# norabelrose/sparse-vae

Hardware: AMD Instinct MI355X
Metric: training tokens/sec + ELBO match vs CPU ref, 512-tok seq, 1/2/4/8 MI355X (higher is better)
Workload: dtype bf16; 1 GPU; c2: TransformerVAE 6L d512 heads 8 seq 512, batch 64/GPU, dense attention, dropout 0.1, fwd+bwd+allreduce+clip+RAdam; model=TransformerVAE-6L-d512, global_batch=64, seq_len=512, parallelism=dp1

## Files before the change

include/svae.h:

```cpp
#ifndef SVAE_H
#define SVAE_H
#include <stdint.h>
#ifdef __cplusplus
extern "C" {
#endif

typedef void* svae_stream_t;

enum svae_epi {
  SVAE_EPI_BF16 = 0,
  SVAE_EPI_F32 = 1,
  SVAE_EPI_F32_ACC = 2,
  SVAE_EPI_F32_ATOMIC = 3,
  SVAE_EPI_GELU = 4,
  SVAE_EPI_GELU_BWD = 5,
  SVAE_EPI_DROPOUT_RESID = 6,
  SVAE_EPI_ROTARY_BF16 = 7,
  SVAE_EPI_CE_STATS = 8,
  SVAE_EPI_CE_PROB = 9,
  SVAE_EPI_ROWSCALE_GATHER = 10
};

typedef struct svae_gemm_desc {
  const void* A;
// ... 9 lines not shown
  const float* resid;
  int64_t ldr;
  void* aux;
  int64_t ldaux;
  float alpha;
  float drop_p;
  uint64_t seed;
  const float* rot_tab;
  int32_t rot_cols, rot_d, rot_seq;
  const int32_t* labels;
  float* label_logit;
  float* a_rowsum;
  const float* k_weight;
  const float* row_a;
  const float* row_b;
  const void* gather;
  int64_t ldg;
  float* delta;
  const float* delta_o32;
  int64_t ld_o32;
  int32_t delta_hd, delta_seq;
} svae_gemm_desc;

int svae_gemm(const svae_gemm_desc* d, svae_stream_t stream);

int svae_gemm_pair(const svae_gemm_desc* d0, const svae_gemm_desc* d1, svae_stream_t stream);

#define SVAE_GROUP_MAX 256
#define SVAE_GROUP_MAX_BLOCKS 1024
int64_t svae_gemm_group_table_bytes(int32_t n);
int svae_gemm_group(const svae_gemm_desc* d, int32_t n, int32_t max_blocks, void* table, void* table_host,
                    int64_t table_bytes, svae_stream_t stream);

int svae_resid_ln_fwd(const float* x, const void* y, int32_t y_dtype, int64_t ldy, float drop_p, uint64_t seed,
                      const float* zrows, int32_t zmod, const float* w, const float* b, float* xo, void* h, float* mean,
                      float* rstd, int32_t rows, int32_t D, svae_stream_t stream);
int svae_layernorm_fwd(const void* x, int32_t x_dtype, const float* w, const float* b, void* y,
                       float* mean, float* rstd, int32_t rows, int32_t D, svae_stream_t stream);
int svae_layernorm_bwd(const void* dy, const void* x, int32_t x_dtype, const float* w, const float* mean,
                       const float* rstd, const float* dres, float* dx, void* dx_bf, float* part,
                       int32_t nblk, int32_t rows, int32_t D, int32_t zero_mod, svae_stream_t stream);
int svae_layernorm_bwd_drop(const void* dy, const void* x, int32_t x_dtype, const float* w, const float* mean,
                            const float* rstd, const float* dres, float* dx, void* dx_bf, float* part, int32_t nblk,
                            int32_t rows, int32_t D, int32_t zero_mod, float bf_drop_p, uint64_t bf_seed,
                            int32_t bf_zero_mod, float* zrow, void* zrow_bf, svae_stream_t stream);
int svae_layernorm_bwd_gelu(const void* dy, const void* x, int32_t x_dtype, const float* w, const float* mean,
                            const float* rstd, const void* gp, void* out_bf, float* part, int32_t nblk, int32_t rows,
                            int32_t D, svae_stream_t stream);
int svae_layernorm_fwd_z(float* x, const float* zrows, int32_t zmod, const float* w, const float* b, void* y,
                         float* mean, float* rstd, int32_t rows, int32_t D, svae_stream_t stream);
int svae_layernorm_nblk(int32_t rows);
#define SVAE_LN_MULTI_MAX 4
int svae_layernorm_fwd_multi(const float* x, const float* const* w, const float* const* b, void* const* y, int32_t n,
                             float* mean, float* rstd, int32_t rows, int32_t D, svae_stream_t stream);
int svae_layernorm_bwd_multi(const void* const* dy, const float* x, const float* const* w, const float* mean,
                             const float* rstd, const float* dres, float* dx, float* const* part, int32_t nblk,
                             int32_t n, int32_t rows, int32_t D, svae_stream_t stream);

int svae_colsum(const void* in, int32_t in_dtype, int32_t rows, int32_t cols, int64_t ld, float* out,
                int32_t accumulate, svae_stream_t stream);

#define SVAE_COLSUM_MAX 8
typedef struct svae_colsum_seg {
  const float* in;
  float* out;
  int64_t ld;
// ... 238 lines not shown
```

sparse-vae_amd/csrc/gemm.hip:

```cpp
#include "common.h"
#include "../../include/svae.h"
#include <string.h>
#include <algorithm>
#include <vector>

using namespace svae;

namespace {

constexpr int BM = 128, BN = 128, BK = 64;
constexpr int TILE_BYTES = BM * BK * 2;

struct GP {
  const bf16* A; const bf16* B;
  long long lda, ldb, sA, sB;
  int M, N, K, splits, kchunk, tiles_n, tiles_m;
  void* C; long long ldc, sC;
  const float* bias;
  const float* resid; long long ldr;
  void* aux; long long ldaux;
  float alpha, drop_p;
  unsigned long long seed;
  const float* rot_tab; int rot_cols, rot_d, rot_seq;
  const int* labels; float* label_logit;
// ... 1406 lines not shown

struct SlabRed {
  const float* slab;
  float* C;
  int M, N;
  long long ldc;
  int splits;
};
__device__ __forceinline__ void slab_reduce_range(const SlabRed& r, int blk, int nblk) {
  const int N4 = r.N / 4;
  const long long total = (long long)r.M * N4, plane = (long long)r.M * r.N;
  for (long long i = (long long)blk * 256 + threadIdx.x; i < total; i += (long long)nblk * 256) {
    const long long m = i / N4;
    const int n = (int)(i - m * N4) * 4;
    const float* src = r.slab + m * r.N + n;
    f32x4 acc = *(const f32x4*)src;
    for (int s = 1; s < r.splits; ++s) acc += *(const f32x4*)(src + s * plane);
    f32x4* dst = (f32x4*)(r.C + m * r.ldc + n);
    *dst = *dst + acc;
  }
}
__global__ __launch_bounds__(256) void slab_reduce_kernel(SlabRed r) { slab_reduce_range(r, blockIdx.x, gridDim.x); }
__global__ __launch_bounds__(256) void slab_reduce2_kernel(SlabRed r0, SlabRed r1, int nb0) {
  if ((int)blockIdx.x < nb0) slab_reduce_range(r0, blockIdx.x, nb0);
  else slab_reduce_range(r1, blockIdx.x - nb0, (int)gridDim.x - nb0);
}
struct alignas(16) SlabRedSlot {
  SlabRed r;
};
__global__ __launch_bounds__(256) void slab_reduce_list_kernel(const SlabRedSlot* __restrict__ list, int n) {
  for (int e = 0; e < n; ++e) {
    const SlabRed r = load_uniform(&list[e].r);
    slab_reduce_range(r, blockIdx.x, gridDim.x);
  }
}

}

static SlabRed slab_red(const svae_gemm_desc* d) {
  return SlabRed{(const float*)d->aux, (float*)d->C, d->M, d->N, (long long)d->ldc, d->splits};
}
static long long slab_blocks(const svae_gemm_desc* d) {
  return std::min(4096LL, ((long long)d->M * (d->N / 4) + 255) / 256);
}
static int launch_slab_reduce(const svae_gemm_desc* d, hipStream_t s) {
  hipLaunchKernelGGL(slab_reduce_kernel, dim3((unsigned)slab_blocks(d)), dim3(256), 0, s, slab_red(d));
  SVAE_LAUNCH_CHECK();
  return SVAE_OK;
}

static int validate_desc(const svae_gemm_desc* d) {
  if (!d || !d->A || !d->B || (!d->C && d->epi != SVAE_EPI_CE_STATS)) return SVAE_EINVAL;
  const bool epi_new = d->epi == SVAE_EPI_CE_PROB || d->epi == SVAE_EPI_ROWSCALE_GATHER;
  if (d->M <= 0 || d->N <= 0 || d->K <= 0 || d->batch <= 0 || d->splits <= 0) return SVAE_EINVAL;
  if ((d->K % 8 && !(d->a_t && d->b_t)) || d->lda % 8 || d->ldb % 8) return SVAE_EINVAL;
  if (d->a_t && d->M % 8) return SVAE_EINVAL;
  if (d->b_t && d->N % 8) return SVAE_EINVAL;
  if (((uintptr_t)d->A | (uintptr_t)d->B) & 15) return SVAE_EINVAL;
  if (d->batch_stride_a % 8 || d->batch_stride_b % 8) return SVAE_EINVAL;
  if (d->epi < 0 || d->epi > SVAE_EPI_ROWSCALE_GATHER) return SVAE_EINVAL;
  if (epi_new && (d->a_t || d->splits != 1 || d->batch != 1 || !d->labels || !d->row_a)) return SVAE_EINVAL;
  if (d->epi == SVAE_EPI_CE_PROB && !d->aux) return SVAE_EINVAL;
  if (d->epi == SVAE_EPI_ROWSCALE_GATHER &&
      (!d->row_b || !d->gather || d->ldg % 8 || ((uintptr_t)d->gather & 15) || d->N % 8))
    return SVAE_EINVAL;
  if (d->k_weight && (!d->a_rowsum || !d->a_t || (d->splits != 1 && !(d->epi == SVAE_EPI_F32_ATOMIC && d->aux))))
// ... 404 lines not shown
  memcpy(img.data(), &h, sizeof(h));
  memcpy(img.data() + o_gp, gp.data(), (size_t)n * sizeof(GPSlot));
  if (!map[0].empty()) memcpy(img.data() + o_ma, map[0].data(), map[0].size() * sizeof(GMap));
  if (!map[1].empty()) memcpy(img.data() + o_mb, map[1].data(), map[1].size() * sizeof(GMap));
  if (!red.empty()) memcpy(img.data() + o_red, red.data(), red.size() * sizeof(SlabRedSlot));
  hipStream_t s = (hipStream_t)stream;
  if (memcmp(table_host, img.data(), (size_t)bytes) != 0) {
    memcpy(table_host, img.data(), (size_t)bytes);
    if (hipMemcpyAsync(table, table_host, (size_t)bytes, hipMemcpyHostToDevice, s) != hipSuccess ||
        hipStreamSynchronize(s) != hipSuccess) {
      memset(table_host, 0, sizeof(GroupHeader));
      return SVAE_ELAUNCH;
    }
  }
  const char* t = (const char*)table;
  const GPSlot* tab = (const GPSlot*)(t + o_gp);
  if (!map[0].empty()) {
    hipLaunchKernelGGL((gemm256_group_kernel<SVAE_EPI_F32_ACC>), dim3((unsigned)map[0].size()), dim3(512), 0, s, tab,
                       (const GMap*)(t + o_ma));
    SVAE_LAUNCH_CHECK();
  }
  if (!map[1].empty()) {
    hipLaunchKernelGGL((gemm256_group_kernel<G3_EPI_SLAB>), dim3((unsigned)map[1].size()), dim3(512), 0, s, tab,
                       (const GMap*)(t + o_mb));
    SVAE_LAUNCH_CHECK();
    const long long rb = std::max(1LL, std::min(2048LL, (red_elems + 255) / 256));
    hipLaunchKernelGGL(slab_reduce_list_kernel, dim3((unsigned)rb), dim3(256), 0, s, (const SlabRedSlot*)(t + o_red),
                       (int)red.size());
    SVAE_LAUNCH_CHECK();
  }
  return SVAE_OK;
}

#ifdef SVAE_STAMPS
extern "C" __attribute__((visibility("default"))) int svae_debug_stamps(unsigned long long* host) {
  return hipMemcpyFromSymbol(host, HIP_SYMBOL(svae_stamps), sizeof(svae_stamps)) == hipSuccess ? 0 : -1;
}
extern "C" __attribute__((visibility("default"))) int svae_debug_rt(unsigned long long* host) {
  return hipMemcpyFromSymbol(host, HIP_SYMBOL(svae_rt), sizeof(svae_rt)) == hipSuccess ? 0 : -1;
}
extern "C" __attribute__((visibility("default"))) int svae_debug_stamps_clear() {
  static unsigned long long zeros[8 * 96 * 3];
  return hipMemcpyToSymbol(HIP_SYMBOL(svae_stamps), zeros, sizeof(zeros)) == hipSuccess ? 0 : -1;
}
#endif
```

sparse-vae_amd/sparse_vae/_native.py:

```python
import ctypes
import os

import torch

_HERE = os.path.dirname(os.path.abspath(__file__))
LIB_PATH = os.environ.get('SVAE_LIB') or os.path.join(_HERE, 'libsvae.so')

c_void_p, c_int32, c_int64, c_float, c_uint64 = (ctypes.c_void_p, ctypes.c_int32, ctypes.c_int64,
                                                  ctypes.c_float, ctypes.c_uint64)
c_fptr = ctypes.c_void_p

EPI_BF16, EPI_F32, EPI_F32_ACC, EPI_F32_ATOMIC, EPI_GELU, EPI_GELU_BWD, EPI_DROPOUT_RESID, \
    EPI_ROTARY_BF16, EPI_CE_STATS, EPI_CE_PROB, EPI_ROWSCALE_GATHER = range(11)

LATENT_L2, LATENT_COSINE, LATENT_KL = range(3)
LATENT_METRICS = {'l2': LATENT_L2, 'cosine': LATENT_COSINE, 'kl': LATENT_KL}
LATENT_MAX_BLOCKS = 1024
TSNE_ROWS_PER_BLOCK, TSNE_TILE_COLS = 512, 256
PAIR_RBF, PAIR_IMQ = range(2)
PAIR_KINDS = {'rbf': PAIR_RBF, 'imq': PAIR_IMQ}
PAIRSUM_TILE_COLS, PAIRSUM_MAX_P, MMD_REDUCE_BLOCKS = 32, 8, 256
KMEANS_MAX_K, KMEANS_TILE_CENTROIDS, KMEANS_SORT_BLOCKS, KMEANS_SEED_BLOCK_ROWS = 1024, 32, 256, 256


# ... 10 lines not shown
        ('bias', c_void_p), ('resid', c_void_p), ('ldr', c_int64),
        ('aux', c_void_p), ('ldaux', c_int64),
        ('alpha', c_float), ('drop_p', c_float), ('seed', c_uint64),
        ('rot_tab', c_void_p), ('rot_cols', c_int32), ('rot_d', c_int32), ('rot_seq', c_int32),
        ('labels', c_void_p), ('label_logit', c_void_p),
        ('a_rowsum', c_void_p),
        ('k_weight', c_void_p), ('row_a', c_void_p), ('row_b', c_void_p), ('gather', c_void_p), ('ldg', c_int64),
        ('delta', c_void_p), ('delta_o32', c_void_p), ('ld_o32', c_int64), ('delta_hd', c_int32), ('delta_seq', c_int32),
    ]


class AttnDesc(ctypes.Structure):
    _fields_ = [
        ('q', c_void_p), ('k', c_void_p), ('v', c_void_p), ('o', c_void_p),
        ('sq', c_int64), ('sk', c_int64), ('sv', c_int64), ('so', c_int64),
        ('bq', c_int64), ('bk', c_int64), ('bv', c_int64), ('bo', c_int64),
        ('key_pad', c_void_p), ('lse', c_void_p),
        ('B', c_int32), ('H', c_int32), ('Lq', c_int32), ('Lk', c_int32), ('hd', c_int32), ('causal', c_int32),
        ('scale', c_float),
        ('dout', c_void_p), ('sdo', c_int64), ('bdo', c_int64),
        ('delta', c_void_p), ('dq', c_void_p), ('bdq', c_int64),
        ('dk', c_void_p), ('dv', c_void_p),
        ('sdk', c_int64), ('sdv', c_int64), ('bdk', c_int64), ('bdv', c_int64),
        ('rot_tab', c_void_p), ('rot_d', c_int32),
        ('o32', c_void_p), ('so32', c_int64), ('bo32', c_int64),
        ('dq_part', c_void_p), ('dq_bf', c_void_p), ('ldq_bf', c_int64),
        ('window', c_int32),
        ('delta_ready', c_int32),
        ('o_lo', c_void_p), ('so_lo', c_int64), ('bo_lo', c_int64),
        ('fwd_ws', c_void_p), ('fwd_ws_elems', c_int64),
    ]


GROUP_MAX = 256
COLSUM_MAX = 8
LN_MULTI_MAX = 4


ZPROJ_MAX = 32


class ZprojSeg(ctypes.Structure):
    _fields_ = [('g', c_void_p), ('W', c_void_p), ('dW', c_void_p), ('db', c_void_p)]


class ZprojFwdSeg(ctypes.Structure):
    _fields_ = [('W', c_void_p), ('bias', c_void_p), ('out', c_void_p)]


class ColsumSeg(ctypes.Structure):
    _fields_ = [('inp', c_void_p), ('out', c_void_p), ('ld', c_int64), ('rows', c_int32), ('cols', c_int32)]


_SIGS = {
    'svae_gemm': [ctypes.POINTER(GemmDesc), c_void_p],
    'svae_gemm_pair': [ctypes.POINTER(GemmDesc), ctypes.POINTER(GemmDesc), c_void_p],
    'svae_gemm_group_table_bytes': [c_int32],
    'svae_gemm_group': [ctypes.POINTER(GemmDesc), c_int32, c_int32, c_void_p, c_void_p, c_int64, c_void_p],
    'svae_resid_ln_fwd': [c_void_p, c_void_p, c_int32, c_int64, c_float, c_uint64, c_void_p, c_int32, c_void_p,
                          c_void_p, c_void_p, c_void_p, c_void_p, c_void_p, c_int32, c_int32, c_void_p],
    'svae_layernorm_fwd': [c_void_p, c_int32, c_void_p, c_void_p, c_void_p, c_void_p, c_void_p, c_int32, c_int32,
                           c_void_p],
    'svae_layernorm_bwd': [c_void_p, c_void_p, c_int32, c_void_p, c_void_p, c_void_p, c_void_p, c_void_p, c_void_p,
                           c_void_p, c_int32, c_int32, c_int32, c_int32, c_void_p],
    'svae_layernorm_bwd_drop': [c_void_p, c_void_p, c_int32, c_void_p, c_void_p, c_void_p, c_void_p, c_void_p,
                                c_void_p, c_void_p, c_int32, c_int32, c_int32, c_int32, c_float, c_uint64, c_int32,
                                c_void_p, c_void_p, c_void_p],
    'svae_layernorm_bwd_gelu': [c_void_p, c_void_p, c_int32, c_void_p, c_void_p, c_void_p, c_void_p, c_void_p,
                                c_void_p, c_int32, c_int32, c_int32, c_void_p],
    'svae_layernorm_nblk': [c_int32],
    'svae_colsum': [c_void_p, c_int32, c_int32, c_int32, c_int64, c_void_p, c_int32, c_void_p],
    'svae_colsum_multi': [c_void_p, c_int32, c_void_p],
    'svae_attn_fwd': [ctypes.POINTER(AttnDesc), c_void_p],
    'svae_attn_bwd': [ctypes.POINTER(AttnDesc), c_void_p],
    'svae_attn_dq_part_elems': [c_int32, c_int32, c_int32, c_int32, c_int32],
    'svae_attn_dq_part_elems_w': [c_int32, c_int32, c_int32, c_int32, c_int32, c_int32],
    'svae_attn_fwd_ws_elems': [c_int32, c_int32, c_int32, c_int32, c_int32, c_int32, c_int32],
    'svae_transpose_blocks': [c_void_p, c_void_p, c_void_p, c_int32, c_int32, c_void_p],
    'svae_dq_finalize': [c_void_p, c_void_p, c_int64, c_int32, c_int32, c_void_p, c_int32, c_void_p],
    'svae_embedding_fwd': [c_void_p, c_void_p, c_void_p, c_void_p, c_int32, c_int32, c_void_p],
    'svae_embedding_fwd_dual': [c_void_p, c_void_p, c_void_p, c_void_p, c_int32, c_int32, c_void_p],
    'svae_embedding_bwd': [c_void_p, c_void_p, c_void_p, c_int32, c_int32, c_void_p],
    'svae_reparam_kl_fwd': [c_void_p, c_void_p, c_uint64, c_void_p, c_void_p, c_void_p, c_void_p, c_void_p,
                            c_void_p, c_int32, c_int32, c_void_p],
    'svae_reparam_kl_bwd': [c_void_p, c_void_p, c_void_p, c_void_p, c_void_p, c_void_p, c_int32, c_int32, c_void_p],
    'svae_ce_finalize': [c_void_p, c_int32, c_void_p, c_void_p, c_int32, c_int32, c_int32, c_int32, c_void_p,
                         c_void_p, c_void_p, c_void_p, c_void_p, c_void_p],
    'svae_ce_weighted_nll': [c_void_p, c_void_p, c_void_p, c_int32, c_int32, c_int32, c_int32, c_void_p, c_void_p,
                             c_void_p],
    'svae_ce_red_ws_elems': [c_int32],
# ... 135 lines not shown
```

sparse-vae_amd/sparse_vae/engine.py:

```python
import math
import os
from collections import OrderedDict

import torch

from . import kernels as K
from ._native import COLSUM_MAX, GROUP_MAX, LN_MULTI_MAX, ZPROJ_MAX
from ._native import EPI_BF16, EPI_F32, EPI_F32_ACC, EPI_GELU, EPI_GELU_BWD, EPI_DROPOUT_RESID, \
    EPI_ROTARY_BF16, EPI_CE_STATS, EPI_F32_ATOMIC, EPI_CE_PROB, EPI_ROWSCALE_GATHER

bf16, f32 = torch.bfloat16, torch.float32
ALIGN = 64
CE_CHUNK_NUMEL = 2 ** 30


def _attn_entries(pre, d, learned):
    out = []
    if learned:
        out.append((pre + 'learned_queries', (1, learned, d)))
        names = ['k_linear', 'v_linear']
    else:
        names = ['q_linear', 'k_linear', 'v_linear']
    out += [(pre + n + '.weight', (d, d)) for n in names]
    out += [(pre + n + '.bias', (d,)) for n in names]
# ... 179 lines not shown
        self.head_mode = os.environ.get('SVAE_HEAD', 'prob')
        assert self.head_mode in ('prob', 'logits'), self.head_mode
        self.dw_group = os.environ.get('SVAE_DW_GROUP', '1') != '0'
        self._dw_jobs = []
        self._dwq = None
        self._dw_names = False
        self._dwg_states, self._dwg_sched = [], {}
        self._zp_pending, self._zp_ctx = [], None
        self._cs_pending = []
        self.ncu = (torch.cuda.get_device_properties(flat.device).multi_processor_count
                    if flat.device.type == 'cuda' else 256)

    def rot(self, L, window=0):
        need = max(L, self.hp.num_latents)
        base = 2 * window * 32 if window else 10000
        t = self._rot.get(base)
        if t is None or t.shape[0] < need:
            t = rotary_table(max(need, 512), self.d, base).to(self.P.device)
            self._rot[base] = t
        return t

    def _ln_fwd(self, name, x, rows, tag, zsplice=None):
        D = self.d
        y = self.ws.get(tag + '.y', (rows, D))
        mean = self.ws.get(tag + '.mean', (rows,), f32)
        rstd = self.ws.get(tag + '.rstd', (rows,), f32)
        if zsplice is not None:
            K.layernorm_fwd_z(x, zsplice[0], zsplice[1], self.P.f(name + '.weight'), self.P.f(name + '.bias'), y, mean,
                              rstd, rows, D)
        else:
            K.layernorm_fwd(x, self.P.f(name + '.weight'), self.P.f(name + '.bias'), y, mean, rstd, rows, D)
        return y, (x, mean, rstd)

    def _ln_bwd(self, name, dy, st, rows, dres, dx, dx_bf=None, bf_drop=None, zsplice=None, gelu=None):
        x, mean, rstd = st
        D = self.d
        wg = self.P.grad[self.P.offsets[name + '.weight'][0]:][:2 * D]
        if len(self._cs_pending) == COLSUM_MAX:
            self.flush_colsum()
        k, n1 = len(self._cs_pending), 1024 * 2 * D
        part = self.ws.get('ln.parts', (COLSUM_MAX * n1,), f32)[k * n1:(k + 1) * n1]
        if gelu is not None:
            K.layernorm_bwd_gelu(dy, x, self.P.f(name + '.weight'), mean, rstd, gelu, dx_bf, wg, rows, D, part,
                                 defer=self._cs_pending)
            return
        K.layernorm_bwd(dy, x, self.P.f(name + '.weight'), mean, rstd, dres, dx, dx_bf, wg, rows, D, part,
                        bf_drop=bf_drop, zsplice=zsplice, defer=self._cs_pending)

    def flush_zproj(self):
        if self._zp_pending:
            z_bf, dz, B, d, Z = self._zp_ctx
            K.zproj_bwd_multi(self._zp_pending, z_bf, dz, B, d, Z)
            self._zp_pending = []

    def flush_colsum(self):
        if self._cs_pending:
            K.colsum_multi(self._cs_pending)
            self._cs_pending = []

    def _job(self, dY, X, wname, rows, n_out, n_in, ldy=None, ldx=None, bias=None):
        bg = None
        if bias is not None:
            off = self.P.offsets[bias][0]
            bg = self.P.grad[off:off + n_out]
        return K.DwJob(dY, X, self.P.g(wname), rows, n_out, n_in, ldy, ldx, bg)

# ... 11 lines not shown
        ncu = self.ncu
        eff = lambda s: tiles * s / (ncu * -(-(tiles * s) // ncu))
        return 2 if tiles >= ncu and eff(2) > eff(1) + 0.1 else 1

    def _dw_pair(self, j0, j1):
        if self._dwq is not None:
            self._dw(j0)
            self._dw(j1)
        else:
            K.linear_dw_pair(j0, j1)

    def _bname(self, name, st):
        return f'{name}.{st["tag"]}' if self._dw_names else name

    def flush_dw(self):
        q, self._dw_jobs = self._dw_jobs, []
        k = 0
        for c in range(0, len(q), GROUP_MAX):
            jobs = q[c:c + GROUP_MAX]
            key = tuple((j.n_out, j.n_in, j.rows) for j in jobs)
            if key not in self._dwg_sched:
                self._dwg_sched[key] = K.group_schedule(key, self.ncu)
            for idx, splits, slab in self._dwg_sched[key]:
                if len(self._dwg_states) <= k:
                    self._dwg_states.append(K.DwGroupState(self.P.device))
                K.linear_dw_group([jobs[i] for i in idx], splits, self._dwg_states[k], slab=slab)
                k += 1

    def _db(self, dY, bname, rows, cols, ld=None):
        off = self.P.offsets[bname][0]
        K.colsum(dY, rows, cols, ld or cols, self.P.grad[off:off + cols])

    def layer_fwd(self, pre, x, B, Sx, L, pad, *, learned=0, cross=False, causal=False, ctx=None, heads, hd,
                  drop_p=0.0, seed=0, tag, out=None, window=0, out_bf=None, zsplice=None, ctx_ln=None):
        d, ws, P = self.d, self.ws, self.P
        rows_x = B * Sx
        rot = self.rot(max(Sx, L), window)
        st = {'pre': pre, 'B': B, 'Sx': Sx, 'L': L, 'learned': learned, 'cross': cross, 'causal': causal,
              'heads': heads, 'hd': hd, 'drop_p': drop_p, 'seed': seed, 'x': x, 'tag': tag, 'window': window}
        a = pre + 'attention.'
        h, st['ln_a'] = self._ln_fwd(pre + 'attn_layer_norm', x, rows_x, tag + '.ln_a', zsplice=zsplice)
        st['h'] = h
        pad_k = pad if Sx == L else None
        if learned:
            Lq = learned
            kv = ws.get(tag + '.kv', (rows_x, 2 * d))
            K.gemm(h, P.w(a + 'k_linear.weight'), kv, rows_x, 2 * d, d, epi=EPI_ROTARY_BF16,
                   bias=P.f(a + 'k_linear.bias'), rot=rot, rot_cols=d, rot_d=d, rot_seq=Sx)
            q = P.w(a + 'learned_queries').view(Lq, d)
            qargs = dict(sq=d, bq=0)
            kt, vt, sk = kv, kv[:, d:], 2 * d
            st['kv'] = kv
        else:
            Lq = Sx
            qkv = ws.get(tag + '.qkv', (rows_x, 3 * d))
            K.gemm(h, P.w(a + 'q_linear.weight'), qkv, rows_x, 3 * d, d, epi=EPI_ROTARY_BF16,
                   bias=P.f(a + 'q_linear.bias'), rot=rot, rot_cols=2 * d, rot_d=d, rot_seq=Sx)
            q = qkv
            qargs = dict(sq=3 * d, bq=Sx * 3 * d)
            kt, vt, sk = qkv[:, d:], qkv[:, 2 * d:], 3 * d
            st['qkv'] = qkv
        rows_q = B * Lq
        O = ws.get(tag + '.O', (rows_q, d))
        Ox = self._o_extra(tag + '.O', rows_q, d, Lq)
        lse = ws.get(tag + '.lse', (B, heads, Lq), f32)
        K.attention(q, kt, vt, O, lse, B=B, H=heads, Lq=Lq, Lk=Sx, hd=hd, so=d, bo=Lq * d, sk=sk, sv=sk,
                    bk=Sx * sk, bv=Sx * sk, key_pad=pad_k, causal=causal, window=window, **Ox, **qargs)
        st.update(O=O, Ox=Ox, lse=lse, Lq=Lq, pad_k=pad_k)
        resid = Lq == Sx
        x1 = ws.get(tag + '.x1', (rows_q, d), f32)
        K.gemm(O, P.w(a + 'output_linear.weight'), x1, rows_q, d, d, epi=EPI_F32,
               bias=P.f(a + 'output_linear.bias'), resid=x if resid else None, ldr=d)
        st['resid'] = resid
        st['x1'] = x1
        xc = x1
        if cross:
            c = pre + 'cross_attention.'
            rows_c = B * L
            if ctx_ln is not None:
                cx, st['ln_ctx'] = ctx_ln
                st['ctx_deferred'] = True
            else:
                cx, st['ln_ctx'] = self._ln_fwd(pre + 'context_layer_norm', ctx, rows_c, tag + '.ln_ctx')
            hq, st['ln_cross'] = self._ln_fwd(pre + 'cross_attn_layer_norm', x1, rows_q, tag + '.ln_cross')
            qc = ws.get(tag + '.qc', (rows_q, d))
            K.gemm(hq, P.w(c + 'q_linear.weight'), qc, rows_q, d, d, epi=EPI_ROTARY_BF16, bias=P.f(c + 'q_linear.bias'),
                   rot=rot, rot_cols=d, rot_d=d, rot_seq=Lq)
            kvc = ws.get(tag + '.kvc', (rows_c, 2 * d))
            K.gemm(cx, P.w(c + 'k_linear.weight'), kvc, rows_c, 2 * d, d, epi=EPI_ROTARY_BF16,
                   bias=P.f(c + 'k_linear.bias'), rot=rot, rot_cols=d, rot_d=d, rot_seq=L)
            Oc = ws.get(tag + '.Oc', (rows_q, d))
            Ocx = self._o_extra(tag + '.Oc', rows_q, d, Lq)
            lsec = ws.get(tag + '.lsec', (B, heads, Lq), f32)
            K.attention(qc, kvc, kvc[:, d:], Oc, lsec, B=B, H=heads, Lq=Lq, Lk=L, hd=hd, sq=d, bq=Lq * d, sk=2 * d,
                        sv=2 * d, bk=L * 2 * d, bv=L * 2 * d, so=d, bo=Lq * d, key_pad=pad, causal=False, **Ocx)
            st['Ocx'] = Ocx
            x2 = ws.get(tag + '.x2', (rows_q, d), f32)
            K.gemm(Oc, P.w(c + 'output_linear.weight'), x2, rows_q, d, d, epi=EPI_F32,
                   bias=P.f(c + 'output_linear.bias'), resid=x1, ldr=d)
            st.update(cx=cx, hq=hq, qc=qc, kvc=kvc, Oc=Oc, lsec=lsec, x2=x2, pad_ctx=pad)
            xc = x2
        h2, st['ln_f'] = self._ln_fwd(pre + 'ffn_layer_norm', xc, rows_q, tag + '.ln_f')
        gprime = ws.get(tag + '.gprime', (rows_q, 4 * d))
        f = ws.get(tag + '.f', (rows_q, 4 * d))
        K.gemm(h2, P.w(pre + 'ffn.0.weight'), f, rows_q, 4 * d, d, epi=EPI_GELU, bias=P.f(pre + 'ffn.0.bias'),
               aux=gprime, ldaux=4 * d)
        out = ws.get(tag + '.out', (rows_q, d), f32) if out is None else out
        K.gemm(f, P.w(pre + 'ffn.2.weight'), out, rows_q, d, 4 * d, epi=EPI_DROPOUT_RESID, resid=xc, ldr=d,
               drop_p=drop_p, seed=seed, aux=out_bf, ldaux=d if out_bf is not None else 0)
        st.update(h2=h2, gprime=gprime, f=f, xc=xc, rows_q=rows_q)
        return out, st

    def _o_extra(self, tag, rows_q, d, Lq):
        return dict(o_lo=self.ws.get(tag + 'lo', (rows_q, d)), so_lo=d, bo_lo=Lq * d)

    def _dq_part(self, B, H, Lq, Lk, hd, window=0):
        n = K.attn_dq_part_elems(B, H, Lq, Lk, hd, window)
        t = self.ws.bufs.get('b.dqpart')
        return t if t is not None and t.numel() >= n else self.ws.get('b.dqpart', (n,), f32)

    def layer_bwd(self, st, dout, dx_out, *, dx_accumulate=False, dctx=None, g2_ready=False, next_drop=None,
                  zsplice=None, next_st=None):
        d, ws, P = self.d, self.ws, self.P
        pre, B, Sx, L, Lq = st['pre'], st['B'], st['Sx'], st['L'], st['Lq']
        heads, hd = st['heads'], st['hd']
        rows_x, rows_q = B * Sx, st['rows_q']
        rot = self.rot(max(Sx, L), st['window'])
        a = pre + 'attention.'
        bn = lambda name: self._bname(name, st)
        self._dwq = self._dw_jobs if self._dw_names else None
        g2 = ws.get(bn('b.g2'), (rows_q, d))
        if not g2_ready:
            K.dropout_bwd_cast(dout, g2, st['drop_p'], st['seed'], rows_q, d)
        dpre = ws.get(bn('b.dpre'), (rows_q, 4 * d))
        K.gemm(g2, P.wT(pre + 'ffn.2.weight', d, 4 * d), dpre, rows_q, 4 * d, d, epi=EPI_GELU_BWD, aux=st['gprime'],
# ... 306 lines not shown
        gp0 = ws.get('h0_gprime', (T, d))
        h0 = ws.get('h0', (T, d))
        K.gemm(xf, P.w('output_layer.0.weight'), h0, T, d, d, epi=EPI_GELU, bias=P.f('output_layer.0.bias'),
               aux=gp0, ldaux=d)
        hh, ln_h = self._ln_fwd('output_layer.2', h0, T, 'head.ln')
        return hh, gp0, h0, ln_h

    def _decode(self, x_emb, zb, padm, B, L, dropout, seed, x_ready=False):
        hp, d, ws, P = self.hp, self.d, self.ws, self.P
        T, Z = B * L, hp.latent_depth
        if self.window and L % 32:
            raise ValueError(f'sparse decoder attention needs seq_len % 32 == 0 (SparseAttention block_size 32, '
                             f'sparse_attention.py:81), got {L}')
        xs = ws.get('x_dec0', (T, d), f32)
        if not x_ready:
            xs.copy_(x_emb)
        xf = ws.get('xf_bf', (T, d))
        dec = []
        zf_batch = d % 8 == 0 and Z <= 1024
        if zf_batch:
            zall = ws.get('zproj_all', (hp.num_layers, B, d), f32)
            segs = [(P.w(f'z_projections.{i}.weight'), P.f(f'z_projections.{i}.bias'), zall[i])
                    for i in range(hp.num_layers)]
            for c0 in range(0, len(segs), ZPROJ_MAX):
                K.zproj_fwd_multi(segs[c0:c0 + ZPROJ_MAX], zb, B, d, Z)
        for i in range(hp.num_layers):
            last = i + 1 == hp.num_layers
            if not zf_batch:
                K.gemm(zb, P.w(f'z_projections.{i}.weight'), xs, B, d, Z, ldc=L * d, epi=EPI_F32,
                       bias=P.f(f'z_projections.{i}.bias'))
            xs, st = self.layer_fwd(f'decoder_layers.{i}.', xs, B, L, L, padm, causal=True, heads=self.H,
                                    hd=self.hd, drop_p=dropout, seed=_mix_seed(seed, i), tag=f'd{i}',
                                    out=ws.get(f'x_dec{i + 1}', (T, d), f32), window=self.window,
                                    out_bf=xf if last else None, zsplice=(zall[i], L) if zf_batch else None)
            dec.append(st)
        return xf, dec

    def reconstruct_f32(self, x_emb, z, pad=None):
        hp, d, P = self.hp, self.d, self.P
        dev = P.device
        B, L = x_emb.shape[0], x_emb.shape[1]
        T, V, Z, H, hd = B * L, hp.vocab_size, hp.latent_depth, self.H, self.hd
        rot = self.rot(L, self.window)
        padm = None
        if pad is not None:
            padm = torch.empty(B, L, dtype=torch.uint8, device=dev)
            padm.copy_(pad)
        x = x_emb.reshape(T, d).clone()
        h = torch.empty(T, d, device=dev)
        qkv = torch.empty(T, 3 * d, device=dev)
        o = torch.empty(T, d, device=dev)
        x1 = torch.empty(T, d, device=dev)
        f = torch.empty(T, 4 * d, device=dev)
        for i in range(hp.num_layers):
            pre = f'decoder_layers.{i}.'
            a = pre + 'attention.'
            K.gemm_f32(z, P.f(f'z_projections.{i}.weight'), x, B, d, Z, ldc=L * d, bias=P.f(f'z_projections.{i}.bias'))
            K.layernorm_fwd_f32(x, P.f(pre + 'attn_layer_norm.weight'), P.f(pre + 'attn_layer_norm.bias'), h, T, d)
            K.gemm_f32(h, P.f(a + 'q_linear.weight'), qkv, T, 3 * d, d, epi=EPI_ROTARY_BF16, bias=P.f(a + 'q_linear.bias'),
                       rot=rot, rot_cols=2 * d, rot_d=d, rot_seq=L)
            K.attention_f32(qkv, qkv[:, d:], qkv[:, 2 * d:], o, B=B, H=H, Lq=L, Lk=L, hd=hd, sq=3 * d, sk=3 * d,
                            sv=3 * d, so=d, bq=L * 3 * d, bk=L * 3 * d, bv=L * 3 * d, bo=L * d, key_pad=padm, causal=True,
                            window=self.window)
            K.gemm_f32(o, P.f(a + 'output_linear.weight'), x1, T, d, d, bias=P.f(a + 'output_linear.bias'), resid=x, ldr=d)
            K.layernorm_fwd_f32(x1, P.f(pre + 'ffn_layer_norm.weight'), P.f(pre + 'ffn_layer_norm.bias'), h, T, d)
            K.gemm_f32(h, P.f(pre + 'ffn.0.weight'), f, T, 4 * d, d, epi=EPI_GELU, bias=P.f(pre + 'ffn.0.bias'))
            K.gemm_f32(f, P.f(pre + 'ffn.2.weight'), x, T, d, 4 * d, resid=x1, ldr=d)
# ... 161 lines not shown
```

sparse-vae_amd/sparse_vae/kernels.py:

```python
import ctypes
import os
from typing import NamedTuple

import torch

from . import _native as N
from ._native import lib, check, ptr, stream

bf16, f32 = torch.bfloat16, torch.float32

_gemm_desc = N.GemmDesc()


def _dev(*ts):
    for t in ts:
        if t is not None and not t.is_cuda:
            raise RuntimeError('libsvae kernels need device tensors (no CPU fallback)')


def gemm(A, B, C, M, N_, K, *, a_t=False, b_t=False, lda=None, ldb=None, ldc=None, epi=N.EPI_BF16, bias=None,
         resid=None, ldr=0, aux=None, ldaux=0, alpha=1.0, splits=1, drop_p=0.0, seed=0, rot=None, rot_cols=0,
         rot_d=0, rot_seq=0, labels=None, label_logit=None, batch=1, sA=0, sB=0, sC=0, a_rowsum=None, k_weight=None,
         row_a=None, row_b=None, gather=None, ldg=0, delta=None, delta_o32=None, ld_o32=0, delta_hd=0, delta_seq=0):
    d = _fill_desc(_gemm_desc, A, B, C, M, N_, K, a_t=a_t, b_t=b_t, lda=lda, ldb=ldb, ldc=ldc, epi=epi, bias=bias,
                   resid=resid, ldr=ldr, aux=aux, ldaux=ldaux, alpha=alpha, splits=splits, drop_p=drop_p, seed=seed,
                   rot=rot, rot_cols=rot_cols, rot_d=rot_d, rot_seq=rot_seq, labels=labels, label_logit=label_logit,
                   batch=batch, sA=sA, sB=sB, sC=sC, a_rowsum=a_rowsum, k_weight=k_weight, row_a=row_a, row_b=row_b,
                   gather=gather, ldg=ldg)
    if delta is not None:
        _dev(delta, delta_o32)
        assert delta.dtype == f32 and delta_o32.dtype == f32 and delta.numel() >= M * (N_ // delta_hd)
    d.delta, d.delta_o32, d.ld_o32 = ptr(delta), ptr(delta_o32), ld_o32
    d.delta_hd, d.delta_seq = delta_hd, delta_seq
    check(lib.svae_gemm(ctypes.byref(d), stream()), 'svae_gemm')


def _fill_desc(d, A, B, C, M, N_, K, *, a_t=False, b_t=False, lda=None, ldb=None, ldc=None, epi=N.EPI_BF16,
               bias=None, resid=None, ldr=0, aux=None, ldaux=0, alpha=1.0, splits=1, drop_p=0.0, seed=0, rot=None,
               rot_cols=0, rot_d=0, rot_seq=0, labels=None, label_logit=None, batch=1, sA=0, sB=0, sC=0,
               a_rowsum=None, k_weight=None, row_a=None, row_b=None, gather=None, ldg=0):
    _dev(A, B, C)
    assert A.dtype == bf16 and B.dtype == bf16
    d.A, d.B = A.data_ptr(), B.data_ptr()
    d.lda = lda if lda is not None else (M if a_t else K)
    d.ldb = ldb if ldb is not None else (N_ if b_t else K)
    d.batch_stride_a, d.batch_stride_b = sA, sB
    d.M, d.N, d.K = M, N_, K
    d.batch, d.splits = batch, splits
    d.a_t, d.b_t = int(a_t), int(b_t)
    d.epi = epi
    d.C = ptr(C)
    d.ldc = ldc if ldc is not None else N_
    d.batch_stride_c = sC
    d.bias = ptr(bias)
    d.resid = ptr(resid)
    d.ldr = ldr
    d.aux = ptr(aux)
    d.ldaux = ldaux
    d.alpha = alpha
    d.drop_p = drop_p
    d.seed = seed & 0xFFFFFFFFFFFFFFFF
    d.rot_tab = ptr(rot)
    d.rot_cols, d.rot_d, d.rot_seq = rot_cols, rot_d, rot_seq
    d.labels = ptr(labels)
    d.label_logit = ptr(label_logit)
    d.a_rowsum = ptr(a_rowsum)
    d.k_weight = ptr(k_weight)
# ... 1002 lines not shown
```

Before: 2.830 million tokens/s.

## Fuse decoder attention output projection with residual add and FFN LayerNorm

Adds a persistent GEMM kernel for N=512 where each block owns full 128x512 output rows. It adds bias and residual, then computes LayerNorm mean and rstd through cross-wave LDS reductions and writes the normalized bf16 activations in the epilogue. In the decoder layers this replaces the separate output-linear GEMM plus LayerNorm launch, saving one pass over the f32 activations and a kernel launch. The cost is a new hand-written GEMM with BK=32 and one block per CU, which may run the matmul itself less efficiently than the existing tuned GEMM.

```diff
diff --git a/include/svae.h b/include/svae.h
--- a/include/svae.h
+++ b/include/svae.h
@@ -65,6 +65,18 @@
 int svae_gemm_group(const svae_gemm_desc* d, int32_t n, int32_t max_blocks, void* table, void* table_host,
                     int64_t table_bytes, svae_stream_t stream);
 
+typedef struct svae_ln_tail {
+  const float* ln_w;
+  const float* ln_b;
+  void* h;
+  float* mean;
+  float* rstd;
+  const float* zrows;
+  int32_t zmod;
+  int32_t max_blocks;
+} svae_ln_tail;
+int svae_gemm_ln(const svae_gemm_desc* d, const svae_ln_tail* t, svae_stream_t stream);
+
 int svae_resid_ln_fwd(const float* x, const void* y, int32_t y_dtype, int64_t ldy, float drop_p, uint64_t seed,
                       const float* zrows, int32_t zmod, const float* w, const float* b, float* xo, void* h, float* mean,
                       float* rstd, int32_t rows, int32_t D, svae_stream_t stream);
diff --git a/sparse-vae_amd/csrc/gemm.hip b/sparse-vae_amd/csrc/gemm.hip
--- a/sparse-vae_amd/csrc/gemm.hip
+++ b/sparse-vae_amd/csrc/gemm.hip
@@ -1462,6 +1462,234 @@
   for (int e = 0; e < n; ++e) {
     const SlabRed r = load_uniform(&list[e].r);
     slab_reduce_range(r, blockIdx.x, gridDim.x);
+  }
+}
+
+constexpr int GL_BK = 32;
+constexpr int GL_TA = 128 * GL_BK * 2;
+constexpr int GL_TB = 512 * GL_BK * 2;
+constexpr int GL_STAGE = GL_TA + GL_TB;
+constexpr int GL_NSTAGE = 3;
+constexpr int GL_SIDE = 3 * 512 * 4 + 128 * 2 * 8 * 4;
+constexpr int GL_PIECES = 5;
+static_assert(8 * 1024 == GL_TA && 8 * 4 * 1024 == GL_TB, "8 waves x (1 + 4) pieces cover a stage exactly");
+static_assert(GL_NSTAGE * GL_STAGE + GL_SIDE <= 160 * 1024, "LDS");
+
+struct LNTail {
+  const float* w; const float* b;
+  bf16* h; float* mean; float* rstd;
+  const float* zrows; int zmod;
+};
+
+__device__ __forceinline__ void gl_piece(int piece, int lane, int& row, int& c) {
+  const int slot = piece * 64 + lane;
+  row = slot >> 2;
+  c = (slot & 3) ^ ((row >> 1) & 3);
+}
+
+__device__ __forceinline__ void gl_issue(const GP& p, int m0, int k0, char* stage, int wave, int offa,
+                                         const int (&offb)[4]) {
+  const int krem = p.K - k0;
+  const u32x4 ra = buffer_rsrc(p.A + (long long)m0 * p.lda + k0, 0x7FFFFFF0u);
+  const u32x4 rb = buffer_rsrc(p.B + k0, 0x7FFFFFF0u);
+  if (krem >= GL_BK && m0 + 128 <= p.M) {
+    dma16_lds(ra, stage + wave * 1024, offa);
+  } else {
+    int row, c;
+    gl_piece(wave, lane_id_fresh(), row, c);
+    const bool ok = row < p.M - m0 && c * 8 < krem;
+    dma16_lds(ra, stage + wave * 1024, ok ? (row * (int)p.lda + c * 8) * 2 : 0x7FFFFFF0);
+  }
+  if (krem >= GL_BK) {
+    dma16x4_lds(rb, stage + GL_TA + wave * 4096, offb[0], offb[1], offb[2], offb[3]);
+  } else {
+    const int lane = lane_id_fresh();
+    int o[4];
+#pragma unroll
+    for (int i = 0; i < 4; ++i) {
+      int row, c;
+      gl_piece(wave * 4 + i, lane, row, c);
+      o[i] = c * 8 < krem ? (row * (int)p.ldb + c * 8) * 2 : 0x7FFFFFF0;
+    }
+    dma16x4_lds(rb, stage + GL_TA + wave * 4096, o[0], o[1], o[2], o[3]);
+  }
+}
+
+template <int EPI, bool LN>
+__global__ __launch_bounds__(512, 1) void gemm_ln_kernel(GP p, LNTail t) {
+  __shared__ __attribute__((aligned(16))) char ring[GL_NSTAGE * GL_STAGE + GL_SIDE];
+  float* sbias = (float*)(ring + GL_NSTAGE * GL_STAGE);
+  float* slw = sbias + 512;
+  float* slb = sbias + 1024;
+  float* sstat = sbias + 1536;
+  const int tid = threadIdx.x, lane = tid & 63;
+  const int wave = __builtin_amdgcn_readfirstlane(tid >> 6);
+  const int g = lane >> 4, li = lane & 15;
+  const int step_m = (int)gridDim.x * 128;
+  int m0 = (int)blockIdx.x * 128;
+  if (m0 >= p.M) return;
+  sbias[tid] = p.bias ? p.bias[tid] : 0.f;
+  if constexpr (LN) {
+    slw[tid] = t.w[tid];
+    slb[tid] = t.b[tid];
+  }
+  const int nk = (p.K + GL_BK - 1) / GL_BK;
+  int offa, offb[4];
+  {
+    int row, c;
+    gl_piece(wave, lane, row, c);
+    offa = (row * (int)p.lda + c * 8) * 2;
+#pragma unroll
+    for (int i = 0; i < 4; ++i) {
+      gl_piece(wave * 4 + i, lane, row, c);
+      offb[i] = (row * (int)p.ldb + c * 8) * 2;
+    }
+  }
+  int pm0 = m0, pkt = 0, is = 0, ahead = 0;
+  auto issue = [&]() {
+    if (pm0 >= p.M) return;
+    gl_issue(p, pm0, pkt * GL_BK, ring + is * GL_STAGE, wave, offa, offb);
+    is = is + 1 == GL_NSTAGE ? 0 : is + 1;
+    ++ahead;
+    if (++pkt == nk) {
+      pkt = 0;
+      pm0 += step_m;
+    }
+  };
+  issue();
+  issue();
+  int cs = 0;
+  bool drained = false;
+  const int aoff = li * 64 + ((g ^ ((li >> 1) & 3)) << 4);
+  for (; m0 < p.M; m0 += step_m) {
+    f32x4 acc[8][4];
+#pragma unroll
+    for (int i = 0; i < 8; ++i)
+#pragma unroll
+      for (int j = 0; j < 4; ++j) acc[i][j] = (f32x4){0.f, 0.f, 0.f, 0.f};
+    for (int kt = 0; kt < nk; ++kt) {
+      if (ahead >= 2 && !drained) asm volatile("s_waitcnt vmcnt(%0)" ::"n"(GL_PIECES) : "memory");
+      else asm volatile("s_waitcnt vmcnt(0)" ::: "memory");
+      drained = false;
+      __builtin_amdgcn_s_barrier();
+      issue();
+      const char* la = ring + cs * GL_STAGE + aoff;
+      const char* lb = la + GL_TA + wave * 64 * 64;
+      bf16x8 af[8], bfr[4];
+#pragma unroll
+      for (int i = 0; i < 8; ++i) af[i] = *(const bf16x8*)(la + i * 1024);
+#pragma unroll
+      for (int j = 0; j < 4; ++j) bfr[j] = *(const bf16x8*)(lb + j * 1024);
+#pragma unroll
+      for (int i = 0; i < 8; ++i)
+#pragma unroll
+        for (int j = 0; j < 4; ++j) acc[i][j] = mfma16(bfr[j], af[i], acc[i][j]);
+      cs = cs + 1 == GL_NSTAGE ? 0 : cs + 1;
+      --ahead;
+    }
+    drained = true;
+    const int nb = wave * 64;
+    f32x4 b4[4];
+    if constexpr (EPI != SVAE_EPI_DROPOUT_RESID) {
+#pragma unroll
+      for (int j = 0; j < 4; ++j) b4[j] = *(const f32x4*)(sbias + nb + j * 16 + 4 * g);
+    }
+    const bool ld = p.resid != nullptr;
+    auto ld_row = [&](int i, f32x4 (&r)[4]) {
+      const int m = m0 + i * 16 + li;
+#pragma unroll
+      for (int j = 0; j < 4; ++j)
+        r[j] = (ld && m < p.M) ? *(const f32x4*)(p.resid + (long long)m * p.ldr + nb + j * 16 + 4 * g)
+                               : (f32x4){0.f, 0.f, 0.f, 0.f};
+    };
+    f32x4 cur[4], nxt[4];
+    ld_row(0, cur);
+#pragma unroll
+    for (int i = 0; i < 8; ++i) {
+      if (i + 1 < 8) ld_row(i + 1, nxt);
+      const int rl = i * 16 + li, m = m0 + rl;
+      f32x4 x[4];
+#pragma unroll
+      for (int j = 0; j < 4; ++j) {
+        if constexpr (EPI == SVAE_EPI_DROPOUT_RESID) {
+          x[j] = acc[i][j];
+          if (p.drop_p > 0.f) dropout4(p, x[j], m, nb + j * 16 + 4 * g);
+        } else {
+          x[j] = acc[i][j] + b4[j];
+        }
+        x[j] += cur[j];
+      }
+      if (t.zrows && m < p.M && m % t.zmod == 0) {
+        const float* z = t.zrows + (long long)(m / t.zmod) * 512 + nb + 4 * g;
+#pragma unroll
+        for (int j = 0; j < 4; ++j) x[j] = *(const f32x4*)(z + j * 16);
+      }
+      store_rows_f32((float*)p.C, p.ldc, m0 + i * 16, p.M, nb, 512, x, g, li);
+      if constexpr (EPI == SVAE_EPI_DROPOUT_RESID) {
+        if (p.aux) store_rows_bf16<false>((bf16*)p.aux, p.ldaux, m0 + i * 16, p.M, nb, 512, x, g, li);
+      }
+      if constexpr (LN) {
+        float s = 0.f;
+#pragma unroll
+        for (int j = 0; j < 4; ++j) {
+          acc[i][j] = x[j];
+          s += (x[j][0] + x[j][1]) + (x[j][2] + x[j][3]);
+        }
+        s = sum_x16_x32(s);
+        if (g == 0) sstat[rl * 16 + wave] = s;
+      }
+      if (i + 1 < 8) {
+#pragma unroll
+        for (int j = 0; j < 4; ++j) cur[j] = nxt[j];
+      }
+    }
+    if constexpr (LN) {
+      auto row_total = [&](int i, int which) {
+        const float* s = sstat + (i * 16 + li) * 16 + which * 8;
+        const f32x4 a = *(const f32x4*)s, b = *(const f32x4*)(s + 4);
+        return ((a[0] + a[1]) + (a[2] + a[3])) + ((b[0] + b[1]) + (b[2] + b[3]));
+      };
+      asm volatile("s_waitcnt lgkmcnt(0)" ::: "memory");
+      __builtin_amdgcn_s_barrier();
+      float mean[8], rstd[8];
+#pragma unroll
+      for (int i = 0; i < 8; ++i) {
+        mean[i] = row_total(i, 0) * (1.0f / 512.0f);
+        float sq = 0.f;
+#pragma unroll
+        for (int j = 0; j < 4; ++j)
+#pragma unroll
+          for (int e = 0; e < 4; ++e) {
+            const float d = acc[i][j][e] - mean[i];
+            sq += d * d;
+          }
+        sq = sum_x16_x32(sq);
+        if (g == 0) sstat[(i * 16 + li) * 16 + 8 + wave] = sq;
+      }
+      asm volatile("s_waitcnt lgkmcnt(0)" ::: "memory");
+      __builtin_amdgcn_s_barrier();
+      f32x4 w4[4], l4[4];
+#pragma unroll
+      for (int j = 0; j < 4; ++j) {
+        w4[j] = *(const f32x4*)(slw + nb + j * 16 + 4 * g);
+        l4[j] = *(const f32x4*)(slb + nb + j * 16 + 4 * g);
+      }
+#pragma unroll
+      for (int i = 0; i < 8; ++i) {
+        rstd[i] = rsqrtf(row_total(i, 1) * (1.0f / 512.0f) + 1e-5f);
+        f32x4 y[4];
+#pragma unroll
+        for (int j = 0; j < 4; ++j)
+#pragma unroll
+          for (int e = 0; e < 4; ++e) y[j][e] = (acc[i][j][e] - mean[i]) * rstd[i] * w4[j][e] + l4[j][e];
+        store_rows_bf16<false>(t.h, 512, m0 + i * 16, p.M, nb, 512, y, g, li);
+        const int m = m0 + i * 16 + li;
+        if (wave == 0 && g == 0 && m < p.M) {
+          t.mean[m] = mean[i];
+          t.rstd[m] = rstd[i];
+        }
+      }
+    }
   }
 }
 
@@ -1932,6 +2160,37 @@
   return SVAE_OK;
 }
 
+SVAE_EXPORT int svae_gemm_ln(const svae_gemm_desc* d, const svae_ln_tail* t, svae_stream_t stream) {
+  if (!d || !t) return SVAE_EINVAL;
+  if (const int rc = validate_desc(d)) return rc;
+  if (d->N != 512 || d->a_t || d->b_t || d->batch != 1 || d->splits != 1 || d->alpha != 1.0f) return SVAE_EINVAL;
+  if (d->epi != SVAE_EPI_F32 && d->epi != SVAE_EPI_DROPOUT_RESID) return SVAE_EINVAL;
+  if (d->a_rowsum || d->k_weight || d->delta) return SVAE_EINVAL;
+  if ((d->epi == SVAE_EPI_F32 && d->aux) || (d->epi == SVAE_EPI_DROPOUT_RESID && d->bias)) return SVAE_EINVAL;
+  if (!(d->drop_p >= 0.f && d->drop_p < 1.f)) return SVAE_EINVAL;
+  if (d->ldc % 4 || d->ldc < 512 || ((uintptr_t)d->C & 15) || d->lda < d->K || d->ldb < d->K || d->lda > (1 << 22) ||
+      d->ldb > (1 << 20) || d->M > (1 << 30) || (d->resid && d->ldr < 512) || (d->aux && d->ldaux < 512))
+    return SVAE_EINVAL;
+  const bool ln = t->ln_w != nullptr;
+  if (ln && (!t->ln_b || !t->h || !t->mean || !t->rstd || ((uintptr_t)t->h & 15) || ((uintptr_t)t->ln_w & 3) ||
+             ((uintptr_t)t->ln_b & 3) || ((uintptr_t)t->mean & 3) || ((uintptr_t)t->rstd & 3)))
+    return SVAE_EINVAL;
+  if (!ln && (d->epi != SVAE_EPI_F32 || t->ln_b || t->h || t->mean || t->rstd)) return SVAE_EINVAL;
+  if (t->zrows && (t->zmod <= 0 || ((uintptr_t)t->zrows & 15))) return SVAE_EINVAL;
+  if (t->max_blocks < 0) return SVAE_EINVAL;
+  GP p;
+  fill_gp(d, p);
+  const LNTail lt{t->ln_w, t->ln_b, (bf16*)t->h, t->mean, t->rstd, t->zrows, t->zmod};
+  const int tiles = (d->M + 127) / 128;
+  const dim3 grid((unsigned)std::min(tiles, t->max_blocks ? t->max_blocks : device_cus()));
+  hipStream_t s = (hipStream_t)stream;
+  if (!ln) hipLaunchKernelGGL((gemm_ln_kernel<SVAE_EPI_F32, false>), grid, dim3(512), 0, s, p, lt);
+  else if (d->epi == SVAE_EPI_F32) hipLaunchKernelGGL((gemm_ln_kernel<SVAE_EPI_F32, true>), grid, dim3(512), 0, s, p, lt);
+  else hipLaunchKernelGGL((gemm_ln_kernel<SVAE_EPI_DROPOUT_RESID, true>), grid, dim3(512), 0, s, p, lt);
+  SVAE_LAUNCH_CHECK();
+  return SVAE_OK;
+}
+
 #ifdef SVAE_STAMPS
 extern "C" __attribute__((visibility("default"))) int svae_debug_stamps(unsigned long long* host) {
   return hipMemcpyFromSymbol(host, HIP_SYMBOL(svae_stamps), sizeof(svae_stamps)) == hipSuccess ? 0 : -1;
diff --git a/sparse-vae_amd/sparse_vae/_native.py b/sparse-vae_amd/sparse_vae/_native.py
--- a/sparse-vae_amd/sparse_vae/_native.py
+++ b/sparse-vae_amd/sparse_vae/_native.py
@@ -66,6 +66,11 @@
     ]
 
 
+class LnTail(ctypes.Structure):
+    _fields_ = [('ln_w', c_void_p), ('ln_b', c_void_p), ('h', c_void_p), ('mean', c_void_p), ('rstd', c_void_p),
+                ('zrows', c_void_p), ('zmod', c_int32), ('max_blocks', c_int32)]
+
+
 GROUP_MAX = 256
 COLSUM_MAX = 8
 LN_MULTI_MAX = 4
@@ -90,6 +95,7 @@
     'svae_gemm': [ctypes.POINTER(GemmDesc), c_void_p],
     'svae_gemm_pair': [ctypes.POINTER(GemmDesc), ctypes.POINTER(GemmDesc), c_void_p],
     'svae_gemm_group_table_bytes': [c_int32],
+    'svae_gemm_ln': [ctypes.POINTER(GemmDesc), c_void_p, c_void_p],
     'svae_gemm_group': [ctypes.POINTER(GemmDesc), c_int32, c_int32, c_void_p, c_void_p, c_int64, c_void_p],
     'svae_resid_ln_fwd': [c_void_p, c_void_p, c_int32, c_int64, c_float, c_uint64, c_void_p, c_int32, c_void_p,
                           c_void_p, c_void_p, c_void_p, c_void_p, c_void_p, c_int32, c_int32, c_void_p],
diff --git a/sparse-vae_amd/sparse_vae/engine.py b/sparse-vae_amd/sparse_vae/engine.py
--- a/sparse-vae_amd/sparse_vae/engine.py
+++ b/sparse-vae_amd/sparse_vae/engine.py
@@ -235,6 +235,14 @@
             K.layernorm_fwd(x, self.P.f(name + '.weight'), self.P.f(name + '.bias'), y, mean, rstd, rows, D)
         return y, (x, mean, rstd)
 
+    def _gemm_ln_fwd(self, name, tag, A, W, C, rows, Kd, **kw):
+        D = self.d
+        y = self.ws.get(tag + '.y', (rows, D))
+        mean = self.ws.get(tag + '.mean', (rows,), f32)
+        rstd = self.ws.get(tag + '.rstd', (rows,), f32)
+        K.gemm_ln(A, W, C, rows, Kd, ln=(self.P.f(name + '.weight'), self.P.f(name + '.bias'), y, mean, rstd), **kw)
+        return y, (C, mean, rstd)
+
     def _ln_bwd(self, name, dy, st, rows, dres, dx, dx_bf=None, bf_drop=None, zsplice=None, gelu=None):
         x, mean, rstd = st
         D = self.d
@@ -312,7 +320,7 @@
         K.colsum(dY, rows, cols, ld or cols, self.P.grad[off:off + cols])
 
     def layer_fwd(self, pre, x, B, Sx, L, pad, *, learned=0, cross=False, causal=False, ctx=None, heads, hd,
-                  drop_p=0.0, seed=0, tag, out=None, window=0, out_bf=None, zsplice=None, ctx_ln=None):
+                  drop_p=0.0, seed=0, tag, out=None, window=0, out_bf=None, zsplice=None, ctx_ln=None, fuse_ln=False):
         d, ws, P = self.d, self.ws, self.P
         rows_x = B * Sx
         rot = self.rot(max(Sx, L), window)
@@ -349,8 +357,14 @@
         st.update(O=O, Ox=Ox, lse=lse, Lq=Lq, pad_k=pad_k)
         resid = Lq == Sx
         x1 = ws.get(tag + '.x1', (rows_q, d), f32)
-        K.gemm(O, P.w(a + 'output_linear.weight'), x1, rows_q, d, d, epi=EPI_F32,
-               bias=P.f(a + 'output_linear.bias'), resid=x if resid else None, ldr=d)
+        fuse_ln_f = fuse_ln and d == K.GEMM_LN_N and resid and not cross
+        if fuse_ln_f:
+            h2, st['ln_f'] = self._gemm_ln_fwd(pre + 'ffn_layer_norm', tag + '.ln_f', O, P.w(a + 'output_linear.weight'),
+                                               x1, rows_q, d, epi=EPI_F32, bias=P.f(a + 'output_linear.bias'),
+                                               resid=x, ldr=d)
+        else:
+            K.gemm(O, P.w(a + 'output_linear.weight'), x1, rows_q, d, d, epi=EPI_F32,
+                   bias=P.f(a + 'output_linear.bias'), resid=x if resid else None, ldr=d)
         st['resid'] = resid
         st['x1'] = x1
         xc = x1
@@ -380,7 +394,8 @@
                    bias=P.f(c + 'output_linear.bias'), resid=x1, ldr=d)
             st.update(cx=cx, hq=hq, qc=qc, kvc=kvc, Oc=Oc, lsec=lsec, x2=x2, pad_ctx=pad)
             xc = x2
-        h2, st['ln_f'] = self._ln_fwd(pre + 'ffn_layer_norm', xc, rows_q, tag + '.ln_f')
+        if not fuse_ln_f:
+            h2, st['ln_f'] = self._ln_fwd(pre + 'ffn_layer_norm', xc, rows_q, tag + '.ln_f')
         gprime = ws.get(tag + '.gprime', (rows_q, 4 * d))
         f = ws.get(tag + '.f', (rows_q, 4 * d))
         K.gemm(h2, P.w(pre + 'ffn.0.weight'), f, rows_q, 4 * d, d, epi=EPI_GELU, bias=P.f(pre + 'ffn.0.bias'),
@@ -753,7 +768,8 @@
             xs, st = self.layer_fwd(f'decoder_layers.{i}.', xs, B, L, L, padm, causal=True, heads=self.H,
                                     hd=self.hd, drop_p=dropout, seed=_mix_seed(seed, i), tag=f'd{i}',
                                     out=ws.get(f'x_dec{i + 1}', (T, d), f32), window=self.window,
-                                    out_bf=xf if last else None, zsplice=(zall[i], L) if zf_batch else None)
+                                    out_bf=xf if last else None, zsplice=(zall[i], L) if zf_batch else None,
+                                    fuse_ln=True)
             dec.append(st)
         return xf, dec
 
diff --git a/sparse-vae_amd/sparse_vae/kernels.py b/sparse-vae_amd/sparse_vae/kernels.py
--- a/sparse-vae_amd/sparse_vae/kernels.py
+++ b/sparse-vae_amd/sparse_vae/kernels.py
@@ -33,6 +33,36 @@
     d.delta, d.delta_o32, d.ld_o32 = ptr(delta), ptr(delta_o32), ld_o32
     d.delta_hd, d.delta_seq = delta_hd, delta_seq
     check(lib.svae_gemm(ctypes.byref(d), stream()), 'svae_gemm')
+
+
+_ln_tail = N.LnTail()
+GEMM_LN_N = 512
+
+
+def gemm_ln(A, B, C, M, K, *, epi, ln=None, bias=None, resid=None, ldr=0, aux=None, ldaux=0, drop_p=0.0, seed=0,
+            lda=None, ldb=None, ldc=None, zsplice=None, max_blocks=0):
+    d = _fill_desc(_gemm_desc, A, B, C, M, GEMM_LN_N, K, lda=lda, ldb=ldb, ldc=ldc, epi=epi, bias=bias, resid=resid,
+                   ldr=ldr, aux=aux, ldaux=ldaux, drop_p=drop_p, seed=seed)
+    t = _ln_tail
+    if ln is not None:
+        w, b, h, mean, rstd = ln
+        _dev(w, b, h, mean, rstd)
+        assert w.dtype == f32 and b.dtype == f32 and mean.dtype == f32 and rstd.dtype == f32 and h.dtype == bf16
+        assert w.numel() == GEMM_LN_N and b.numel() == GEMM_LN_N and w.is_contiguous() and b.is_contiguous()
+        assert h.is_contiguous() and h.numel() >= M * GEMM_LN_N and mean.numel() >= M and rstd.numel() >= M
+        t.ln_w, t.ln_b, t.h, t.mean, t.rstd = ptr(w), ptr(b), ptr(h), ptr(mean), ptr(rstd)
+    else:
+        t.ln_w = t.ln_b = t.h = t.mean = t.rstd = None
+    if zsplice is not None:
+        zrows, zmod = zsplice
+        _dev(zrows)
+        assert zrows.dtype == f32 and zrows.is_contiguous() and zmod > 0
+        assert zrows.numel() >= -(-M // zmod) * GEMM_LN_N
+        t.zrows, t.zmod = ptr(zrows), int(zmod)
+    else:
+        t.zrows, t.zmod = None, 0
+    t.max_blocks = int(max_blocks)
+    check(lib.svae_gemm_ln(ctypes.byref(d), ctypes.addressof(t), stream()), 'svae_gemm_ln')
 
 
 def _fill_desc(d, A, B, C, M, N_, K, *, a_t=False, b_t=False, lda=None, ldb=None, ldc=None, epi=N.EPI_BF16,
```

Result: no change. 2.839 million tokens/s (median of 6 runs) (+0.3%).
